# omkuprin7/ldpc-simulator

Hardware: AMD Instinct MI355X
Metric: decoded codewords/s + info-bits/s at fixed (N, rate, max_iter, Eb/N0) (higher is better)
Workload: dtype f64

## Files before the change

### ldpc-simulator_amd/csrc/ldpc_api.cpp

```cpp
#include <hip/hip_runtime.h>

#include <algorithm>
#include <cfloat>
#include <climits>
#include <cstdarg>
#include <cstdio>
#include <cstring>
#include <mutex>
#include <string>
#include <vector>

#include "ldpc_internal.h"
#include "mc_stats_host.h"
#include "rate_match_host.h"
#include "spa_device.h"

using ldpc::DevGraph;
using ldpc::DevState;
using ldpc::PhysRule;
using ldpc::PhysTile;
using ldpc::kTile;

static thread_local std::string g_last_error;

// ... 65 lines not shown
    uint32_t *ord_keys = nullptr;
    int *ord_vals = nullptr, *ord = nullptr;
    int64_t ord_cap = 0;
    void *ord_tmp = nullptr;
    size_t ord_tmp_bytes = 0;
    DevState st{};
    bool ms_on = false;
    int ms_max_failed = 0;
    unsigned long long *ms_buf = nullptr;
    size_t ms_words = 0;
    long long *ms_slots = nullptr;
    int *ms_tile = nullptr;
    int ms_state = 0;
    int ms_points = 0, ms_T = 0, ms_run_failed = 0;
    ldpc::FrameChannel chan{};
    std::vector<int32_t> rm_punct, rm_short;
    ldpc::RateMatchTables rm_tab;
    uint32_t *rm_dev = nullptr;
    bool rm_stale = false;
    bool prof = false;
    struct Span {
        int kind;
        hipEvent_t a, b;
    };
    std::vector<Span> spans;
    std::vector<hipEvent_t> pool;
};

namespace {

constexpr size_t kLdsLimit = 160 * 1024 - 1024;

int tile_scratch_rows(const DevGraph &g) { return g.ef == 8 ? ldpc::tile8_scratch_per_tile(g) : 2; }

template <int W = ldpc::kSubWaves>
std::vector<int> sub_p3_deps(int m, const int *row_ptr, const int *col_idx, bool drop_last = false) {
    std::vector<int> dep((size_t)m * W, 1);
    auto spans = [&](int r, long long lo[W], long long hi[W], bool ne[W]) {
        const int beg = row_ptr[r];
        const int deg = std::max(0, row_ptr[r + 1] - beg - (drop_last ? 1 : 0)), C = (deg + W - 1) / W;
        long long prev = -1;
        int last = -1;
        for (int w = 0; w < W; ++w) {
            const int cnt = std::max(0, std::min(deg - w * C, C));
            ne[w] = cnt > 0;
            if (!ne[w]) continue;
            lo[w] = prev + 1;
            hi[w] = prev = col_idx[beg + w * C + cnt - 1];
            last = w;
        }
        if (last >= 0) hi[last] = LLONG_MAX;
        return last >= 0;
    };
    long long plo[W], phi[W], lo[W], hi[W];
    bool pne[W], ne[W];
    bool prev_any = m > 0 && spans(0, plo, phi, pne);
    for (int r = 1; r < m; ++r) {
        spans(r, lo, hi, ne);
        for (int w = 0; w < W; ++w) {
            if (!ne[w]) continue;
            int vlo = W, vhi = -1;
            for (int v = 0; v < W; ++v)
                if (!prev_any || (pne[v] && plo[v] <= hi[w] && lo[w] <= phi[v])) {
                    vlo = std::min(vlo, v);
                    vhi = std::max(vhi, v);
                }
// ... 1 lines not shown
        }
        std::copy(lo, lo + W, plo);
        std::copy(hi, hi + W, phi);
        std::copy(ne, ne + W, pne);
        prev_any = std::any_of(ne, ne + W, [](bool b) { return b; });
    }
    return dep;
}

int require_gpu() {
    int n = 0;
    if (hipGetDeviceCount(&n) != hipSuccess || n <= 0)
        return ldpc_fail(LDPC_EDEVICE, "no HIP device visible: the SPA decoder runs only on the GPU");
    return LDPC_OK;
}

template <class T>
int dev_alloc(T **p, size_t count) {
    *p = nullptr;
    if (count == 0) return LDPC_OK;
    hipError_t e = hipMalloc((void **)p, count * sizeof(T));
    if (e != hipSuccess) {
        *p = nullptr;
        return ldpc_fail(LDPC_ENOMEM, "hipMalloc(%zu bytes) failed: %s", count * sizeof(T), hipGetErrorString(e));
    }
    return LDPC_OK;
}

int ensure_messages(ldpc_decoder *d) {
    if (d->E) return LDPC_OK;
    const DevGraph &G = d->g->dg;
    const size_t cap = (size_t)d->cap_tiles * kTile;
    int rc = dev_alloc(&d->E, cap * (size_t)G.nnz + (size_t)ldpc::kEPadEdges * kTile);
    if (!rc) rc = dev_alloc(&d->T, (size_t)d->nslots * G.max_row_deg * kTile);
    if (rc) {
        (void)hipFree(d->E);
        d->E = nullptr;
    }
    return rc;
}

int ensure_pbits(ldpc_decoder *d, const DevGraph &P) {
    if (d->pbits) return LDPC_OK;
    const size_t mw = (size_t)(P.m + 31) / 32, mw32 = (mw + 31) / 32;
    return dev_alloc(&d->pbits, (size_t)d->cap_tiles * (mw + mw32) * kTile);
}

int ensure_phys_tile(ldpc_decoder *d, const DevGraph &P) {
    const size_t cap = (size_t)d->cap_tiles * kTile;
    const int64_t need = (int64_t)(cap * (size_t)P.nnz);
    if (d->pE_cap < need) {
        (void)hipFree(d->pE);
        d->pE = nullptr;
        d->pE_cap = 0;
        if (int rc = dev_alloc(&d->pE, (size_t)need)) return rc;
        d->pE_cap = need;
    }
    if (!d->pL && dev_alloc(&d->pL, cap * (size_t)d->g->dg.n)) return LDPC_ENOMEM;
    if (!d->pLam && dev_alloc(&d->pLam, cap * (size_t)d->g->dg.n)) return LDPC_ENOMEM;
    if (!d->pbad && dev_alloc(&d->pbad, 2 * cap)) return LDPC_ENOMEM;
    if (!d->pzb && dev_alloc(&d->pzb, cap * (size_t)((d->g->dg.n + 7) / 8))) return LDPC_ENOMEM;
    return LDPC_OK;
}

PhysTile phys_tile(ldpc_decoder *d) {
    const DevGraph &G = d->g->dg;
    uint32_t *wpar = d->pbits ? d->pbits + (size_t)d->cap_tiles * ((G.m + 31) / 32) * kTile : nullptr;
// ... 183 lines not shown
        if (e == hipSuccess) {
            const bool last = it + 1 == max_iter;
            if (edge)
                e = timed(d, LDPC_K_VN_EDGE, s, [&] {
                    return ldpc::launch_vn_edge_decode(G, st, it, last, nllr, d->tzb, d->tcnt, d->tbad, s);
                });
            else if (cols)
                e = timed(d, LDPC_K_VN_COLS, s, [&] {
                    return ldpc::launch_vn_cols_decode(G, st, it, last, nllr, d->tzb, d->tcnt, s);
                });
            else
                e = timed(d, LDPC_K_VN, s, [&] { return ldpc::launch_vn(G, st, it, max_iter, nllr, s); });
        }
        if (e == hipSuccess && poll && it + 1 < max_iter && (it < 4 || (it + 1) % 4 == 0)) {
            int running = 0;
            e = hipMemcpyAsync(&running, d->pactive + it, sizeof(int), hipMemcpyDeviceToHost, s);
            if (e == hipSuccess) e = hipStreamSynchronize(s);
            if (e == hipSuccess && running == 0) break;
        }
    }
    return hip(e);
}

int scratch_slots() { return 4096; }


size_t workspace_bytes(const DevGraph &g, int cap_tiles) {
    const size_t cap = (size_t)cap_tiles * kTile;
    const size_t kw = (size_t)((g.k + 31) / 32);
    size_t b = 0;
    b += cap * (size_t)g.nnz * 8;
    const size_t slots = ldpc::use_tile(g) ? std::max(scratch_slots(), cap_tiles * tile_scratch_rows(g)) : scratch_slots();
    b += slots * g.max_row_deg * kTile * 8;
    b += 4 * (kRareHead + (size_t)cap_tiles * g.m * 4);
    b += 2 * cap * (size_t)g.n * 8;
    b += (7 * cap + cap_tiles) * 4;
    b += cap * kw * 4;
    b += 2 * cap * (size_t)g.n * 8;
    b += cap * (size_t)g.n;
    b += cap * ((size_t)(g.n + 31) / 32) * 4 + 2 * cap * 4;
    return b;
}

}

extern "C" {

const char *ldpc_last_error(void) { return g_last_error.c_str(); }
int ldpc_abi_version(void) { return LDPC_ABI_VERSION; }

int ldpc_device_count(void) {
    int n = 0;
    if (hipGetDeviceCount(&n) != hipSuccess) return 0;
    return n;
}

namespace {

int check_csr(const char *fn, int32_t m, int32_t n, const int32_t *row_ptr, const int32_t *col_idx, int *max_row,
              int *min_row) {
    if (m <= 0 || n <= 0 || m > n || !row_ptr || !col_idx)
        return ldpc_fail(LDPC_EINVAL, "%s: bad shape m=%d n=%d", fn, m, n);
    if (row_ptr[0] != 0) return ldpc_fail(LDPC_EINVAL, "%s: row_ptr[0] != 0", fn);
    const int64_t nnz = row_ptr[m];
    if (nnz <= 0 || nnz > (int64_t)(INT32_MAX / kTile) || (int64_t)n > (int64_t)(INT32_MAX / kTile))
        return ldpc_fail(LDPC_ERANGE, "%s: nnz=%lld outside 32-bit tile indexing", fn, (long long)nnz);
// ... 1728 lines not shown
```

### ldpc-simulator_amd/csrc/spa_device.h

```cpp
#pragma once
#include <hip/hip_runtime.h>
#include <cstdint>

namespace ldpc {

constexpr int kTile = 64;

constexpr int kSubWaves = 16;
constexpr int kEPadEdges = 128;

struct DevGraph {
    int m, n, k, nnz;
    int max_row_deg, max_col_deg;
    int std_form;
    int ira;
    const int *row_ptr;
    const int *col_idx;
    const int *csc_ptr;
    const int *csc_edge;
    const int *csc_row;
    const uint32_t *a_packed;
    const int *p3dep;
    const int *p3dep8;
    int ef;
// ... 32 lines not shown
    uint32_t *pbits;
    uint32_t *wpar;
    int cap;
    uint8_t *zb;
};

hipError_t launch_reset(const DevGraph &g, const DevState &st, hipStream_t s);
hipError_t launch_load_llr(const DevGraph &g, const DevState &st, const double *llr, hipStream_t s);
hipError_t launch_cn(const DevGraph &g, const DevState &st, int it, hipStream_t s, bool stream = false);
bool use_cn_row(const DevGraph &g);
hipError_t launch_cn_rare(const DevGraph &g, const DevState &st, int it, hipStream_t s, bool stream = false);
hipError_t launch_vn(const DevGraph &g, const DevState &st, int it, int max_iter, bool nllr, hipStream_t s,
                     unsigned long long *stream_ctr = nullptr);
size_t tile_lds_bytes(const DevGraph &g);
const char *tile_kernel_name(const DevGraph &g);
bool use_tile(const DevGraph &g);
hipError_t launch_tile(const DevGraph &g, const DevState &st, int max_iter, bool nllr, hipStream_t s);
bool use_tile_stream(const DevGraph &g);
hipError_t launch_tile_stream(const DevGraph &g, const DevState &st, int max_iter, bool nllr, uint64_t seed,
                              int snr_point, double sigma, int64_t frame0, int64_t total, unsigned long long *next,
                              unsigned long long *ctr, int64_t handoff, hipStream_t s);
bool tile8_applies(const DevGraph &g);
bool tile8_pair_fits(const DevGraph &g);
size_t tile8_lds_bytes(const DevGraph &g);
int tile8_scratch_per_tile(const DevGraph &g);
hipError_t launch_tile8(const DevGraph &g, const DevState &st, int max_iter, bool nllr, hipStream_t s);
size_t tile8_stream_lds_bytes(const DevGraph &g);
hipError_t launch_tile8_stream(const DevGraph &g, const DevState &st, int max_iter, bool nllr, uint64_t seed,
                               int snr_point, double sigma, int64_t frame0, int64_t total, unsigned long long *next,
                               unsigned long long *ctr, int64_t handoff, hipStream_t s);
size_t tile64_lds_bytes(const DevGraph &g);
int sub_frames(const DevGraph &g);
size_t sub_lds_bytes(const DevGraph &g);
hipError_t launch_tile_sub(const DevGraph &g, const DevState &st, int max_iter, bool nllr, hipStream_t s);
hipError_t launch_tile_sub_stream(const DevGraph &g, const DevState &st, int max_iter, bool nllr, uint64_t seed,
                                  int snr_point, double sigma, int64_t frame0, int64_t total,
                                  unsigned long long *next, unsigned long long *ctr, int64_t handoff, hipStream_t s);
hipError_t launch_stream_init(const DevGraph &g, const DevState &st, hipStream_t s);
hipError_t launch_vn_tail(const DevGraph &g, const DevState &st, int max_iter, bool nllr, uint32_t *zb, int *cnt,
                          unsigned long long *ctr, hipStream_t s);
hipError_t launch_vn_cols_decode(const DevGraph &g, const DevState &st, int it, bool last, bool nllr, uint32_t *zb,
                                 int *cnt, hipStream_t s);
hipError_t launch_tail_exit_decode(const DevGraph &g, const DevState &st, int it, bool last, bool nllr, uint32_t *zb,
                                   int *cnt, int *gbad, hipStream_t s);
int edge_max_deg();
hipError_t launch_cn_edge(const DevGraph &g, const DevState &st, int it, hipStream_t s);
hipError_t launch_vn_edge_decode(const DevGraph &g, const DevState &st, int it, bool last, bool nllr, uint32_t *zb,
                                 int *cnt, int *gbad, hipStream_t s);
int cn_sub_shape(const DevGraph &g);
hipError_t launch_cn_sub(const DevGraph &g, const DevState &st, int it, hipStream_t s, bool stream);
__host__ __device__ inline uint32_t rare_code(int tile_row, uint32_t subs) {
    return (uint32_t)tile_row | (subs << 28);
}
size_t frame_order_temp_bytes(int total);
hipError_t launch_frame_order(const DevGraph &g, uint64_t seed, int snr_point, double sigma, int64_t frame0,
                              int total, uint32_t *keys, int *vals, int *order, void *temp, size_t temp_bytes,
                              hipStream_t s);
__device__ __forceinline__ long long supply_frame(const DevState &st, int64_t frame0, int64_t idx) {
    return (long long)(frame0 + (st.order ? (int64_t)st.order[idx] : idx));
}
hipError_t launch_refill(const DevGraph &g, const DevState &st, uint64_t seed, int snr_point, double sigma,
                         int64_t frame0, int64_t total, unsigned long long *next, hipStream_t s);
hipError_t launch_compact(const DevGraph &g, const DevState &st, int nt, int cap, int *pairs, hipStream_t s);
hipError_t launch_compact_plan(const DevState &st, int nt, int cap, int *pairs, hipStream_t s);
hipError_t launch_finalize(const DevGraph &g, const DevState &st, uint8_t *z, double *post,
                           hipStream_t s);
// ... 166 lines not shown
```

### ldpc-simulator_amd/csrc/tile_sub.hip

```cpp
#include <hip/hip_runtime.h>

#include <cstdint>
#include <cstdlib>

#include "cn_common.h"
#include "frame_source.h"
#include "spa_device.h"
#include "spa_math.h"
#include "tile_common.h"

namespace ldpc {
namespace {

constexpr int kSW = kSubWaves;
#ifdef LDPC_SUB_TIMERS
#define SUB_NT 7
#define SUB_STAMP(v) const uint64_t v = __builtin_amdgcn_s_memtime()
#define SUB_ADD(c, i, a, b) ((c).tm[i] += (b) - (a))
#else
#define SUB_STAMP(v)
#define SUB_ADD(c, i, a, b)
#endif
constexpr size_t kSubLdsMax = 163840;


template <int Q>
struct SubCfg {
    static constexpr int F = kTile / Q;
    static constexpr int K = Q == 4 ? 10 : 8;
};

constexpr int kSR = 4;
__device__ __forceinline__ int sub_wave(int hw) { return (hw & 3) * (kSW / 4) + (hw >> 2); }
typedef unsigned int sub_u2 __attribute__((ext_vector_type(2)));
constexpr uint32_t kSubOOB = 0xfffffff0u;
__device__ __forceinline__ void st_sub_msg(__amdgpu_buffer_rsrc_t r, uint32_t off, double v) {
    __builtin_amdgcn_raw_buffer_store_b64(__builtin_bit_cast(sub_u2, v), r, off, 0, 2 );
}
__device__ __forceinline__ double ld_sub_msg(__amdgpu_buffer_rsrc_t r, uint32_t off) {
    return __builtin_bit_cast(double, __builtin_amdgcn_raw_buffer_load_b64(r, off, 0, 2 ));
}
__device__ __forceinline__ __amdgpu_buffer_rsrc_t sub_rsrc(const void *base, size_t bytes) {
    return __builtin_amdgcn_make_buffer_rsrc(const_cast<void *>(base), (short)0, (int)min(bytes, (size_t)0x7fffffff),
                                            0x00020000);
}

constexpr int kCRing = 3;
struct SubLayout {
    size_t S, math, slot, zb, ib, lane_i, flags, dummy, cidx, total;
// ... 36 lines not shown
    c.cnt = max(0, min(c.deg - wave * C, C));
    c.CS = (C + Q - 1) / Q;
    return c;
}

template <int Q>
struct SubCtx {
    static constexpr int F = SubCfg<Q>::F;
    static constexpr int K = SubCfg<Q>::K;
    const int *__restrict__ col_idx;
    const int *__restrict__ row_ptr;
    double *Eb;
    double *Lb;
    const double *Cb;
    double *Tb;
    size_t tbuf;
    double *S;
    double *dummy;
    double *slot;
    uint32_t *ib;
    uint16_t *cidx;
    int m;
    int *flag, *tinyf, *tseq, *p3row;
    const int *p3dep;
    LdsTanh ttab;
    LdsAtanh ltab;
    AtanhCoef ac;
    bool coef_arg;
    const char *Eu, *Lu, *Cu;
    __amdgpu_buffer_rsrc_t rE;
    uint32_t lo8;
    int k, wave, j, f;
    int ep0;
    bool first, live;
    bool fresh;
    bool verify;
    bool prove;
    int *mdiff;
    int ntiny;
#ifdef LDPC_SUB_TIMERS
    mutable uint64_t tm[SUB_NT];
#endif
};

template <int Q>
__device__ __forceinline__ int sub_nj(const SubCtx<Q> &c, const SubChunk &rc) {
    return max(0, min(rc.cnt - c.j * rc.CS, rc.CS));
}
template <int Q>
__device__ __forceinline__ int sub_edge(const SubCtx<Q> &c, const SubChunk &rc, int i) {
    return rc.c0 + min(c.j * rc.CS + i, rc.cnt - 1);
}
template <int Q>
__device__ __forceinline__ uint32_t sub_off(const SubCtx<Q> &c, int item) {
    return ((uint32_t)item << 9) + c.lo8;
}
template <int Q>
__device__ __forceinline__ double *sub_l(const SubCtx<Q> &c, int col) {
    return (double *)(c.Lu + sub_off(c, col));
}
template <int Q>
__device__ __forceinline__ const double *sub_c(const SubCtx<Q> &c, int col) {
    return (const double *)(c.Cu + sub_off(c, col));
}
template <int Q>
__device__ __forceinline__ int sub_col(const SubCtx<Q> &c, int edge) {
    return *(const int *)((const char *)c.col_idx + ((uint32_t)edge << 2));
}
template <int Q>
__device__ __forceinline__ const uint16_t *sub_lcols(const SubCtx<Q> &c, int r, const SubChunk &rc) {
    return c.cidx + (r % kCRing) * kSW * Q * SubCfg<Q>::K + c.j * rc.CS;
}
template <int Q>
__device__ __forceinline__ uint32_t sub_eoff(const SubCtx<Q> &c, const SubChunk &rc) {
    return ((uint32_t)(rc.c0 + c.j * rc.CS) << 9) + c.lo8;
}
template <int Q>
__device__ __forceinline__ int sub_stage_issue(const SubCtx<Q> &c, int q) {
    const SubChunk rc = sub_chunk(c.row_ptr, min(q, c.m - 1), c.wave, Q);
    const int L = threadIdx.x & 63;
    return sub_col(c, min(max(rc.c0 + min(L, rc.cnt - 1), 0), c.row_ptr[c.m] - 1));
}
template <int Q>
__device__ __forceinline__ void sub_stage_commit(const SubCtx<Q> &c, int q, int v) {
    if (q >= c.m) return;
    constexpr int W = Q * SubCfg<Q>::K;
    __builtin_amdgcn_fence(__ATOMIC_RELEASE, "wavefront");
    if ((int)(threadIdx.x & 63) < W) c.cidx[(q % kCRing) * kSW * W + (threadIdx.x & 63)] = (uint16_t)v;
    __builtin_amdgcn_fence(__ATOMIC_ACQUIRE, "wavefront");
}

template <int Q>
__device__ __forceinline__ bool sub_p1(const SubCtx<Q> &c, int r, const SubChunk &rc, double (&t)[SubCfg<Q>::K]) {
    constexpr int K = SubCfg<Q>::K;
    bool tiny = false;
    const int sv = sub_stage_issue(c, r + 1);
    if (rc.cnt > 0 && c.first) {
        const int njt = c.live ? sub_nj(c, rc) : 0;
        const uint16_t *lc = sub_lcols(c, r, rc);
        int col[K];
#pragma unroll
        for (int i = 0; i < K; ++i) col[i] = lc[i];
#pragma unroll
        for (int i = 0; i < K; ++i) t[i] = ld_l2((const double *)(c.Lu + sub_off(c, col[i])));
#pragma unroll
        for (int i = 0; i < K; ++i) {
            tiny |= i < njt && !(fabs(t[i]) > kTiny);
            t[i] = i < njt ? t[i] : 1.0;
        }
    } else if (rc.cnt > 0) {
        const int nj = sub_nj(c, rc);
        const int njt = c.live ? nj : 0;
        const uint16_t *lc = sub_lcols(c, r, rc);
        const uint32_t eoff = sub_eoff(c, rc);
        const bool noE = c.fresh;
        int col[K];
        double eo[K];
#pragma unroll
        for (int i = 0; i < K; ++i) {
            eo[i] = ld_sub_msg(c.rE, noE ? kSubOOB : eoff + (uint32_t)i * (kTile * sizeof(double)));
            col[i] = lc[i];
        }
#pragma unroll
        for (int i = 0; i < K; ++i) t[i] = ld_l2((const double *)(c.Lu + sub_off(c, col[i])));
#pragma unroll
        for (int i = 0; i < K; ++i) {
            const double M = noE ? t[i] : t[i] - eo[i];
            const double d = M * 0.5;
            double th[1] = {dfrom(dbits(fmin(fabs(d), 17.5)) | (dbits(d) & 0x8000000000000000ull))};
            np_tanh_n<1, LdsTanh, true>(th, c.ttab);
            const double tv = th[0];
            tiny |= i < njt && !(fabs(tv) > kTiny);
            t[i] = i < nj ? tv : 1.0;
        }
    }
    sub_stage_commit(c, r + 1, sv);
    return __ballot(tiny) != 0ull;
}

template <int Q>
__device__ __forceinline__ void sub_tanh_table(const SubCtx<Q> &c, int n, int me, int nthr) {
    for (int col = me; col < n; col += nthr) {
        const double d = *sub_c(c, col) * 0.5;
        double th[1] = {dfrom(dbits(fmin(fabs(d), 17.5)) | (dbits(d) & 0x8000000000000000ull))};
        np_tanh_n<1, LdsTanh, true>(th, c.ttab);
        if (c.live) *sub_l(c, col) = th[0];
    }
}

__device__ __forceinline__ uint32_t p16(uint32_t x, int which) {
    const auto r = __builtin_amdgcn_permlane16_swap(x, x, false, false);
    return which ? r[1] : r[0];
}
__device__ __forceinline__ uint32_t p32(uint32_t x, int which) {
    const auto r = __builtin_amdgcn_permlane32_swap(x, x, false, false);
    return which ? r[1] : r[0];
}
__device__ __forceinline__ double group_up4(double v, int jj) {
    const uint64_t u = dbits(v);
    uint32_t lo = (uint32_t)u, hi = (uint32_t)(u >> 32);
    if (jj == 1) {
        lo = p16(p32(lo, 0), 1);
        hi = p16(p32(hi, 0), 1);
    } else {
        lo = p16(lo, 0);
        hi = p16(hi, 0);
    }
    return dfrom(((uint64_t)hi << 32) | lo);
}


template <int K, int N>
struct SubMul {
    static __device__ __forceinline__ double run(double P, const double (&t)[K], int n) {
        if (n == N) {
#pragma unroll
            for (int i = 0; i < N; ++i) P = P * t[i];
            return P;
        }
// ... 35 lines not shown
#pragma unroll
        for (int jj = 0; jj < Q; ++jj) {
            if (jj * rc.CS < rc.cnt) {
                const double Pl = SubMul<K, K>::run(P, t, rc.CS);
                last = jj;
                if (jj + 1 < Q && (jj + 1) * rc.CS < rc.cnt)
                    P = group_up4(Pl, jj);
                else
                    P = Pl;
            }
        }
    }
    if ((threadIdx.x & 63) == 0) {
        if (c.wave == 0)
            lds_st(c.tinyf + s, tiny ? 1 : 0);
        else if (tiny)
            lds_st(c.tinyf + s, 1);
    }
    if (c.j == last) *sl = P;
    lds_release();
    if ((threadIdx.x & 63) == 0) lds_st(c.flag + s, ep + c.wave + 1);
    __builtin_amdgcn_s_setprio(0);
    SUB_STAMP(h2);
    SUB_ADD(c, 1, h1, h2);
}

template <int Q>
__device__ __forceinline__ void sub_order(const SubCtx<Q> &c, int r) {
    if (r > 0) {
        const int d = ld_table(c.p3dep, r * kSW + c.wave);
        for (int v = d & 0xff; v <= (d >> 8); ++v) wait_ge<false>(c.p3row + v, r);
    }
}
template <int Q>
__device__ __forceinline__ void sub_p3_body(SubCtx<Q> &c, int r, double (&t)[SubCfg<Q>::K]) {
    constexpr int F = SubCfg<Q>::F, K = SubCfg<Q>::K;
    const SubChunk rc = sub_chunk(c.row_ptr, r, c.wave, Q);
    if (rc.deg == 0) return;
    const int s = r & (kSR - 1);
    const int ep = ((c.ep0 + r) & 0x3ffffff) * 32;
    const double chI = *sub_c(c, c.k + r);
    SUB_STAMP(q0);
    wait_flag<false>(c.flag + s, ep + kSW);
    SUB_STAMP(q1);
    SUB_ADD(c, 2, q0, q1);
    const bool tiny_row = uniform(lds_ld(c.tinyf + s)) != 0;
    if (rc.cnt == 0) {
        sub_order(c, r);
        if (tiny_row) {
            c.ntiny += 1;
            if ((threadIdx.x & 63) == 0)
                __hip_atomic_fetch_add(c.tseq, 1, __ATOMIC_RELEASE, __HIP_MEMORY_SCOPE_WORKGROUP);
            wait_flag<false>(c.tseq, c.ntiny * kSW);
        }
        return;
    }
    const double P = c.slot[s * F];
    const int nj = sub_nj(c, rc);
    const uint16_t *lc = sub_lcols(c, r, rc);
    int col[K];
#pragma unroll
    for (int i = 0; i < K; ++i)
        col[i] = lc[i];
    if (!tiny_row) {
        bool big = false;
        const double lim = c.live ? kAtanhIdent : INFINITY;
        if (div_nr_ok(c.live ? P : 1.0)) {
#pragma unroll
            for (int i = 0; i < K; ++i)
                if (i < rc.CS) {
                    t[i] = div_nr(P, t[i]);
                    big |= !(fabs(t[i]) < lim);
                }
        } else {
#pragma unroll
            for (int i = 0; i < K; ++i)
                if (i < rc.CS) {
                    t[i] = P / t[i];
                    big |= !(fabs(t[i]) < lim);
                }
        }
        if (__ballot(big) == 0ull) {
#pragma unroll
            for (int i = 0; i < K; ++i)
                if (i < rc.CS) t[i] = 2.0 * t[i];
        } else {
            const AtanhCoef ac = c.coef_arg ? c.ac : coef_load();
#pragma unroll
            for (int i = 0; i < K; ++i)
                if (i < rc.CS) t[i] = 2.0 * atanh_f(clip_cl(t[i]), c.ltab, ac);
// ... 45 lines not shown
            constexpr int H = (K + 1) / 2;
            bool nx = false;
            const bool open = c.prove && d && (lds_ld(c.mdiff + (threadIdx.x & (F - 1))) & 6) == 0;
            if (__ballot(open) != 0ull) {
#pragma unroll
                for (int h = 0; h < K; h += H) {
                    __builtin_amdgcn_sched_barrier(0);
                    double lo[H];
#pragma unroll
                    for (int i = 0; i < H; ++i)
                        lo[i] = ld_l2((const double *)(c.Lu + sub_off(c, col[min(h + i, K - 1)])));
#pragma unroll
                    for (int i = 0; i < H; ++i)
                        if (h + i < K) {
                            const int q = h + i;
                            nx |= q < njv && dbits(lo[i] - eold[q]) != dbits(lo[i] - t[q]);
                            nx |= q < njv && col[q] >= c.k && dbits(chI + (0.0 + t[q])) != dbits(lo[i]);
                        }
                }
            }
#pragma unroll
            for (int i = 0; i < K; ++i) {
                const bool di = i < njv && dbits(eold[i]) != dbits(t[i]);
                st_sub_msg(c.rE, di ? eoff + (uint32_t)i * (kTile * sizeof(double)) : kSubOOB, t[i]);
            }
            if (d) atomicOr((uint32_t *)c.mdiff + (threadIdx.x & (F - 1)), (nx || !open) ? 3u : 1u);
            if (__ballot(nx) != 0ull && (threadIdx.x & 63) < F) atomicOr((uint32_t *)c.mdiff + (threadIdx.x & 63), 4u);
        }
    } else {
        const uint32_t eoff = sub_eoff(c, rc);
#pragma unroll
        for (int i = 0; i < K; ++i)
            st_sub_msg(c.rE, (i < nj && c.live) ? eoff + (uint32_t)i * (kTile * sizeof(double)) : kSubOOB, t[i]);
    }
    double EnI = 0.0;
    int colI = -1;
    double *sp[K];
#pragma unroll
    for (int i = 0; i < K; ++i) {
        const bool own = i < nj;
        const bool a = own && col[i] < c.k;
        sp[i] = a ? c.S + (size_t)col[i] * F : c.dummy;
        if (own && !a) {
            EnI = t[i];
            colI = col[i];
        }
    }
    SUB_STAMP(q2);
    SUB_ADD(c, 3, q1, q2);
    sub_order(c, r);
    SUB_STAMP(q3);
    SUB_ADD(c, 4, q2, q3);
#pragma unroll
    for (int i = 0; i < K; ++i)
        __hip_atomic_fetch_add(sp[i], t[i], __ATOMIC_RELAXED, __HIP_MEMORY_SCOPE_WORKGROUP);
    if (colI >= 0) {
        const double Lj = chI + (0.0 + EnI);
        if (c.live) *sub_l(c, colI) = Lj;
        if (!(Lj < 0.0)) {
            const int q = colI - c.k;
            atomicOr(c.ib + (q >> 5) * F, 1u << (q & 31));
        }
    }
    SUB_STAMP(q4);
    SUB_ADD(c, 5, q3, q4);
}

template <int Q>
__device__ __forceinline__ void sub_p3(SubCtx<Q> &c, int r, double (&t)[SubCfg<Q>::K]) {
    sub_p3_body<Q>(c, r, t);
    lds_release();
    if ((threadIdx.x & 63) == 0)
        lds_st(c.p3row + c.wave, r + 1);
}
__device__ __forceinline__ void sub_p3_reset(int *p3row) {
    if (threadIdx.x < kSW) p3row[threadIdx.x] = 0;
}
__device__ __forceinline__ int sub_epoch0(int pass, int m) {
    return (int)(((uint32_t)pass * (uint32_t)m) & 0x3ffffffu);
}

template <int Q>
__device__ __forceinline__ void sub_body(SubCtx<Q> &c, int r, int m, double (&tcur)[SubCfg<Q>::K], bool ycur,
                                         double (&toth)[SubCfg<Q>::K], bool &yoth) {
    if (r < m) sub_hop(c, r, tcur, ycur);
    if (r >= 1) sub_p3<Q>(c, r - 1, toth);
    SUB_STAMP(p0);
    if (r + 1 < m) yoth = sub_p1<Q>(c, r + 1, sub_chunk(c.row_ptr, r + 1, c.wave, Q), toth);
    SUB_STAMP(p1);
    SUB_ADD(c, 6, p0, p1);
}

template <int Q>
__global__ __launch_bounds__(64 * kSW, 1) void tile_sub_kernel(DevGraph g, DevState st, int max_iter, int nllr,
                                                               const int *__restrict__ col_idx,
                                                               const int *__restrict__ row_ptr, AtanhCoef ac, int fp) {
    constexpr int F = SubCfg<Q>::F, K = SubCfg<Q>::K;
    extern __shared__ __attribute__((aligned(16))) unsigned char lds[];
    __shared__ int pdiffl[F], mdiffl[F];
    const SubLayout ly = sub_layout(g.k, g.m, F);
    double *S = (double *)(lds + ly.S);
    MathLds &mlds = *(MathLds *)(lds + ly.math);
    uint32_t *zb = (uint32_t *)(lds + ly.zb);
    uint32_t *ib = (uint32_t *)(lds + ly.ib);
    int *bad = (int *)(lds + ly.lane_i);
    int *cntl = bad + F;
    int *livel = cntl + F;
    int *flags = (int *)(lds + ly.flags);
    const int kw = (g.k + 31) >> 5, mw = (g.m + 31) >> 5;
    const int tile = blockIdx.x / Q, sub = blockIdx.x % Q;
    if (tile >= st.ntiles) return;

    fill_math_lds(mlds);
    for (int i = threadIdx.x; i < g.k * F; i += blockDim.x) S[i] = 0.0;
    for (int i = threadIdx.x; i < (kw + mw) * F; i += blockDim.x) zb[i] = 0u;
    for (int i = threadIdx.x; i < 2 * F; i += blockDim.x) bad[i] = 0;
    if (threadIdx.x < 2 * kSR) flags[threadIdx.x] = -1;
    if (threadIdx.x >= 2 * kSR && threadIdx.x < 2 * kSR + 2 + kSW) flags[threadIdx.x] = 0;
    const int lane = threadIdx.x & 63;
    const int wave = uniform(sub_wave(threadIdx.x >> 6));
    const int j = lane / F, f = lane % F;
    const int fr = tile * kTile + sub * F + f;
    if (wave == 0 && j == 0) {
        livel[f] = st.done[fr] == 0 ? 1 : 0;
        pdiffl[f] = 0;
        mdiffl[f] = 0;
    }
    __syncthreads();
    if (!st.tile_active[tile]) return;
// ... 10 lines not shown
    const size_t lo = (size_t)sub * F + f;
    c.Eb = st.E + (size_t)tile * g.nnz * kTile + lo;
    c.Lb = st.L + (size_t)tile * g.n * kTile + lo;
    c.Cb = st.ch + (size_t)tile * g.n * kTile + lo;
    c.Eu = (const char *)(st.E + (size_t)tile * g.nnz * kTile);
    c.rE = sub_rsrc(c.Eu, (size_t)g.nnz * kTile * sizeof(double));
    c.Lu = (const char *)(st.L + (size_t)tile * g.n * kTile);
    c.Cu = (const char *)(st.ch + (size_t)tile * g.n * kTile);
    c.lo8 = (uint32_t)lo * 8u;
    c.Tb = st.T + (size_t)blockIdx.x * 2 * g.max_row_deg * F + f;
    c.tbuf = (size_t)g.max_row_deg * F;
    c.S = S + f;
    c.dummy = (double *)(lds + ly.dummy) + f;
    c.slot = (double *)(lds + ly.slot) + f;
    c.ib = ib + f;
    c.cidx = (uint16_t *)(lds + ly.cidx) + wave * Q * K;
    c.m = g.m;
    c.flag = flags;
    c.tinyf = flags + kSR;
    c.tseq = flags + 2 * kSR;
    c.p3row = flags + 2 * kSR + 2;
    c.p3dep = g.p3dep;
    c.ttab = LdsTanh{mlds.tanh};
    c.ltab = LdsAtanh{mlds.atanh};
    c.coef_arg = false;
    c.ac = ac;
    c.k = g.k;
    c.wave = wave;
    c.j = j;
    c.f = f;
    c.ntiny = 0;
    c.fresh = false;
    c.mdiff = mdiffl;
#ifdef LDPC_SUB_TIMERS
    for (int i = 0; i < SUB_NT; ++i) c.tm[i] = 0;
#endif
    const int m = g.m;
    const int nthr = kSW * Q;
    const int me = wave * Q + j;

    int ctl = 1, vnext = 1, vgap = 1;
    const bool fpn = (fp & 2) != 0;
    if (max_iter > 0) {
        c.live = livel[f] != 0;
        sub_tanh_table<Q>(c, g.n, me, nthr);
        __builtin_amdgcn_fence(__ATOMIC_RELEASE, "agent");
        __syncthreads();
    }
    for (int it = 0; it < max_iter; ++it) {
        c.first = it == 0;
        c.live = livel[f] != 0;
        c.ep0 = sub_epoch0(it, m);
        const bool verify = fp != 0 && it >= vnext && (ctl & 2) != 0;
        c.verify = verify;
        c.prove = verify && fpn;
        double tA[K], tB[K];
        bool yA = false, yB = false;
        if (m > 0) {
            sub_stage_commit(c, 0, sub_stage_issue(c, 0));
            yA = sub_p1<Q>(c, 0, sub_chunk(row_ptr, 0, wave, Q), tA);
        }
        for (int r = 0; r <= m; r += 2) {
            sub_body<Q>(c, r, m, tA, yA, tB, yB);
            if (r + 1 <= m) sub_body<Q>(c, r + 1, m, tB, yB, tA, yA);
        }
        __syncthreads();
        sub_p3_reset(c.p3row);

        int my_cnt = 0;
        bool pd = false;
        for (int col = me; col < g.k; col += nthr) {
            double *sp = c.S + (size_t)col * F;
            const double Sj = *sp;
            *sp = 0.0;
            const double chj = *sub_c(c, col);
            const double Lj = chj + Sj;
            if (nllr || fp) {
                const double ap = c.first ? chj : ld_l2(sub_l(c, col));
                if (nllr) my_cnt += (fabs(Lj) <= 7.0 && ap * Lj < 0.0) ? 1 : 0;
                pd |= dbits(ap) != dbits(Lj);
            }
            if (c.live) *sub_l(c, col) = Lj;
            if (!(Lj < 0.0)) atomicOr(zb + (col >> 5) * F + f, 1u << (col & 31));
        }
        if (nllr && my_cnt) atomicAdd(cntl + f, my_cnt);
        if (fp && pd && c.live) atomicOr((uint32_t *)pdiffl + f, 1u);
        __syncthreads();

        uint32_t acc = 0u;
        for (int r = me; r < m; r += nthr) {
            const uint32_t *ar = g.a_packed + (size_t)r * kw;
            uint32_t par = ib[(r >> 5) * F + f] >> (r & 31);
            for (int w = 0; w < kw; ++w) par += __builtin_popcount(ar[w] & zb[w * F + f]);
            acc |= par & 1u;
        }
        if (acc) atomicOr((uint32_t *)bad + f, 1u);
        __syncthreads();

        if (wave == 0) {
            bool still = false, fixed = false, proven = false;
            if (j == 0 && c.live) {
                if (nllr) {
                    const int cn = cntl[f];
                    st.nllr_cnt[fr] = cn;
                    if (st.nllr_hist)
                        st.nllr_hist[(size_t)fr * st.hist_stride + it] = g.k > 0 ? (double)cn / g.k : 0.0;
                }
                if (bad[f] == 0) {
                    st.done[fr] = 1;
                    st.conv[fr] = it;
                    st.status[fr] = 0;
// ... 14 lines not shown
                    proven = mdiffl[f] != 0;
                } else {
                    still = true;
                }
            }
            const unsigned long long any = __ballot(still);
            const unsigned long long trig = __ballot(still && fp && pdiffl[f] == 0);
            const int nfix = __popcll(__ballot(fixed));
            const unsigned long long nprv = __ballot(proven);
            if (j == 0) {
                livel[f] = still ? 1 : 0;
                bad[f] = 0;
                cntl[f] = 0;
                pdiffl[f] = 0;
                mdiffl[f] = 0;
            }
            if (lane == 0) {
                flags[2 * kSR + 1] = (any != 0ull ? 1 : 0) | (trig != 0ull ? 2 : 0) | (nfix ? 4 : 0) | (nprv != 0ull ? 8 : 0);
                if (nfix) {
                    atomicAdd(&st.fp_count[0], (unsigned long long)nfix);
                    atomicAdd(&st.fp_count[1], (unsigned long long)nfix * (unsigned long long)(max_iter - 1 - it));
                }
            }
        }
        for (int i = threadIdx.x; i < (kw + mw) * F; i += blockDim.x) zb[i] = 0u;
        __syncthreads();
        ctl = uniform(flags[2 * kSR + 1]);
        if (!(ctl & 1)) break;
        if (verify && !(ctl & 4)) {
            vnext = it + 1 + vgap;
            vgap *= 2;
        }
    }
    count_rare_rows(st, c.tseq, kSW);
#ifdef LDPC_SUB_TIMERS
    if ((blockIdx.x == 0 || blockIdx.x == 777) && (threadIdx.x & 63) == 0)
        printf("SUB b=%d w=%d hopw=%llu hop=%llu p3f=%llu p3m=%llu p3o=%llu p3s=%llu p1=%llu\n", (int)blockIdx.x,
               c.wave, (unsigned long long)c.tm[0], (unsigned long long)c.tm[1], (unsigned long long)c.tm[2],
               (unsigned long long)c.tm[3], (unsigned long long)c.tm[4], (unsigned long long)c.tm[5],
               (unsigned long long)c.tm[6]);
#endif
}

template <int Q>
__global__ __launch_bounds__(64 * kSW, 1) void tile_sub_stream_kernel(
    DevGraph g, DevState st, int max_iter, int nllr, const int *__restrict__ col_idx,
    const int *__restrict__ row_ptr, AtanhCoef ac, uint64_t seed, int snr_point, double sigma, int64_t frame0,
    int64_t total, unsigned long long *next, unsigned long long *ctr, int64_t handoff) {
    constexpr int F = SubCfg<Q>::F, K = SubCfg<Q>::K;
    extern __shared__ __attribute__((aligned(16))) unsigned char lds[];
    __shared__ int itl[F], freshl[F];
    __shared__ long long gidx[F];
    __shared__ int nref;
    const SubLayout ly = sub_layout(g.k, g.m, F);
    double *S = (double *)(lds + ly.S);
    MathLds &mlds = *(MathLds *)(lds + ly.math);
    uint32_t *zb = (uint32_t *)(lds + ly.zb);
    uint32_t *ib = (uint32_t *)(lds + ly.ib);
    int *bad = (int *)(lds + ly.lane_i);
    int *cntl = bad + F;
    int *livel = cntl + F;
    int *flags = (int *)(lds + ly.flags);
    const int kw = (g.k + 31) >> 5, mw = (g.m + 31) >> 5;
    const int tile = blockIdx.x / Q, sub = blockIdx.x % Q;
    if (tile >= st.ntiles) return;

    fill_math_lds(mlds);
    for (int i = threadIdx.x; i < g.k * F; i += blockDim.x) S[i] = 0.0;
    for (int i = threadIdx.x; i < (kw + mw) * F; i += blockDim.x) zb[i] = 0u;
    for (int i = threadIdx.x; i < 2 * F; i += blockDim.x) bad[i] = 0;
    if (threadIdx.x < 2 * kSR) flags[threadIdx.x] = -1;
    if (threadIdx.x >= 2 * kSR && threadIdx.x < 2 * kSR + 2 + kSW) flags[threadIdx.x] = 0;
    const int lane = threadIdx.x & 63;
    const int wave = uniform(sub_wave(threadIdx.x >> 6));
// ... 11 lines not shown
    c.col_idx = col_idx;
    c.row_ptr = row_ptr;
    const size_t lo = (size_t)lane64;
    c.Eb = st.E + (size_t)tile * g.nnz * kTile + lo;
    c.Lb = st.L + (size_t)tile * g.n * kTile + lo;
    c.Cb = st.ch + (size_t)tile * g.n * kTile + lo;
    c.Eu = (const char *)(st.E + (size_t)tile * g.nnz * kTile);
    c.rE = sub_rsrc(c.Eu, (size_t)g.nnz * kTile * sizeof(double));
    c.Lu = (const char *)(st.L + (size_t)tile * g.n * kTile);
    c.Cu = (const char *)(st.ch + (size_t)tile * g.n * kTile);
    c.lo8 = (uint32_t)lo * 8u;
    c.Tb = st.T + (size_t)blockIdx.x * 2 * g.max_row_deg * F + f;
    c.tbuf = (size_t)g.max_row_deg * F;
    c.S = S + f;
    c.dummy = (double *)(lds + ly.dummy) + f;
    c.slot = (double *)(lds + ly.slot) + f;
    c.ib = ib + f;
    c.cidx = (uint16_t *)(lds + ly.cidx) + wave * Q * K;
    c.m = g.m;
    c.flag = flags;
    c.tinyf = flags + kSR;
    c.tseq = flags + 2 * kSR;
    c.p3row = flags + 2 * kSR + 2;
    c.p3dep = g.p3dep;
    c.ttab = LdsTanh{mlds.tanh};
    c.ltab = LdsAtanh{mlds.atanh};
    c.coef_arg = kStreamCoefArg;
    c.ac = ac;
    c.k = g.k;
    c.wave = wave;
    c.j = j;
    c.f = f;
    c.ntiny = 0;
    c.first = false;
    c.verify = false;
    c.prove = false;
    c.mdiff = nullptr;
    const int m = g.m;
    const int nthr = kSW * Q;
    const int me = wave * Q + j;
    const uint32_t *Ut = st.ubits + (size_t)tile * kw * kTile + lane64;

    for (int pass = 0;; ++pass) {
        if (wave == 0) {
            int stop = 0;
            if (handoff > 0 && lane == 0) {
                const long long nx = (long long)__hip_atomic_load(next, __ATOMIC_RELAXED, __HIP_MEMORY_SCOPE_AGENT);
                const long long fin = (long long)__hip_atomic_load(ctr, __ATOMIC_RELAXED, __HIP_MEMORY_SCOPE_AGENT);
                stop = nx >= total && total - fin <= handoff ? 1 : 0;
            }
            stop = uniform(stop);
            if (stop) want = false;
            const unsigned long long w = __ballot(want);
            bool have = false;
            if (w != 0ull) {
                const int first = __ffsll((long long)w) - 1;
                unsigned long long base = 0ull;
                if (lane == first) base = atomicAdd(next, (unsigned long long)__popcll(w));
                base = __shfl(base, first);
                const unsigned long long below = lane ? (w & (~0ull >> (64 - lane))) : 0ull;
                const int64_t idx = (int64_t)(base + (unsigned long long)__popcll(below));
                have = want && idx < total;
                if (slot_lane) gidx[f] = have ? supply_frame(st, frame0, idx) : -1ll;
                if (want) {
                    livel[f] = have ? 1 : 0;
                    freshl[f] = have ? 1 : 0;
                    itl[f] = 0;
// ... 108 lines not shown
template <int Q>
size_t sub_lds_bytes_q(const DevGraph &g) {
    constexpr int F = SubCfg<Q>::F, K = SubCfg<Q>::K;
    if (!g.std_form || !g.a_packed || g.k <= 0 || g.max_row_deg > kSW * Q * K || Q * K > 64 || g.n > 65535)
        return 0;
    const size_t b = sub_layout(g.k, g.m, F).total;
    return b + 2 * F * sizeof(int) <= kSubLdsMax ? b : 0;
}

}

int sub_frames(const DevGraph &g) { return sub_lds_bytes_q<4>(g) ? 16 : 0; }
size_t sub_lds_bytes(const DevGraph &g) { return sub_lds_bytes_q<4>(g); }

hipError_t launch_tile_sub_stream(const DevGraph &g, const DevState &st, int max_iter, bool nllr, uint64_t seed,
                                  int snr_point, double sigma, int64_t frame0, int64_t total,
                                  unsigned long long *next, unsigned long long *ctr, int64_t handoff, hipStream_t s) {
    const size_t lds = sub_lds_bytes_q<4>(g);
    if (!lds || !g.a_packed || !st.ubits || 2 * st.ntiles > st.nslots ||
        lds + 2 * 16 * sizeof(int) + 16 * sizeof(long long) + 16 > kSubLdsMax)
        return hipErrorInvalidValue;
    tile_sub_stream_kernel<4><<<st.ntiles * 4, 64 * kSW, lds, s>>>(g, st, max_iter, nllr ? 1 : 0, g.col_idx, g.row_ptr,
                                                                   kAtanhCoef, seed, snr_point, sigma, frame0, total,
                                                                   next, ctr, handoff);
    return hipGetLastError();
}

hipError_t launch_tile_sub(const DevGraph &g, const DevState &st, int max_iter, bool nllr, hipStream_t s) {
    const size_t lds = sub_lds_bytes(g);
    if (!lds || 2 * st.ntiles > st.nslots) return hipErrorInvalidValue;
    const char *e = getenv("LDPC_FIXED_POINT");
    const char *en = getenv("LDPC_FP_NEXT");
    const int fp = (!e || atoi(e) != 0) ? (1 | ((!en || atoi(en) != 0) ? 2 : 0)) : 0;
    tile_sub_kernel<4><<<st.ntiles * 4, 64 * kSW, lds, s>>>(g, st, max_iter, nllr ? 1 : 0, g.col_idx, g.row_ptr,
                                                            kAtanhCoef, fp);
    return hipGetLastError();
}

}
```

Before: 125,800.

## Split first decoder iteration into a pass0 kernel with row-product prepass

Adds a separate pass0 kernel that runs iteration 0 of the sub-tile decoder. Before the row sweep, a prepass computes per-row products of tanh values and rare-row flags into a global scratch area. Iteration 0 then consumes these precomputed products through a specialized row loop that skips the flag waits and overlaps the next row's loads with the current row's stores. The main kernel resumes from iteration 1 using a control handoff value stored in global memory. This costs an extra kernel launch, additional global scratch allocation, and more code paths that must stay numerically consistent with the original.

```diff
diff --git a/ldpc-simulator_amd/csrc/ldpc_api.cpp b/ldpc-simulator_amd/csrc/ldpc_api.cpp
--- a/ldpc-simulator_amd/csrc/ldpc_api.cpp
+++ b/ldpc-simulator_amd/csrc/ldpc_api.cpp
@@ -121,6 +121,9 @@
 constexpr size_t kLdsLimit = 160 * 1024 - 1024;
 
 int tile_scratch_rows(const DevGraph &g) { return g.ef == 8 ? ldpc::tile8_scratch_per_tile(g) : 2; }
+size_t sub_p0_total(const DevGraph &g, int cap_tiles) {
+    return g.ef == kTile && ldpc::sub_frames(g) == 16 ? (size_t)cap_tiles * 4 * ldpc::sub_p0_doubles(g.m) : 0;
+}
 
 template <int W = ldpc::kSubWaves>
 std::vector<int> sub_p3_deps(int m, const int *row_ptr, const int *col_idx, bool drop_last = false) {
@@ -188,7 +191,7 @@
     const DevGraph &G = d->g->dg;
     const size_t cap = (size_t)d->cap_tiles * kTile;
     int rc = dev_alloc(&d->E, cap * (size_t)G.nnz + (size_t)ldpc::kEPadEdges * kTile);
-    if (!rc) rc = dev_alloc(&d->T, (size_t)d->nslots * G.max_row_deg * kTile);
+    if (!rc) rc = dev_alloc(&d->T, (size_t)d->nslots * G.max_row_deg * kTile + sub_p0_total(G, d->cap_tiles));
     if (rc) {
         (void)hipFree(d->E);
         d->E = nullptr;
@@ -438,6 +441,7 @@
     b += cap * (size_t)g.nnz * 8;
     const size_t slots = ldpc::use_tile(g) ? std::max(scratch_slots(), cap_tiles * tile_scratch_rows(g)) : scratch_slots();
     b += slots * g.max_row_deg * kTile * 8;
+    b += sub_p0_total(g, cap_tiles) * 8;
     b += 4 * (kRareHead + (size_t)cap_tiles * g.m * 4);
     b += 2 * cap * (size_t)g.n * 8;
     b += (7 * cap + cap_tiles) * 4;
diff --git a/ldpc-simulator_amd/csrc/spa_device.h b/ldpc-simulator_amd/csrc/spa_device.h
--- a/ldpc-simulator_amd/csrc/spa_device.h
+++ b/ldpc-simulator_amd/csrc/spa_device.h
@@ -88,6 +88,10 @@
 size_t tile64_lds_bytes(const DevGraph &g);
 int sub_frames(const DevGraph &g);
 size_t sub_lds_bytes(const DevGraph &g);
+__host__ __device__ inline size_t sub_p0_doubles(int m) { return (size_t)m * 16 + ((size_t)m + 2) / 2; }
+__host__ __device__ inline double *sub_p0(const DevGraph &g, const DevState &st) {
+    return st.T + (size_t)st.nslots * g.max_row_deg * kTile;
+}
 hipError_t launch_tile_sub(const DevGraph &g, const DevState &st, int max_iter, bool nllr, hipStream_t s);
 hipError_t launch_tile_sub_stream(const DevGraph &g, const DevState &st, int max_iter, bool nllr, uint64_t seed,
                                   int snr_point, double sigma, int64_t frame0, int64_t total,
diff --git a/ldpc-simulator_amd/csrc/tile_sub.hip b/ldpc-simulator_amd/csrc/tile_sub.hip
--- a/ldpc-simulator_amd/csrc/tile_sub.hip
+++ b/ldpc-simulator_amd/csrc/tile_sub.hip
@@ -14,7 +14,7 @@
 
 constexpr int kSW = kSubWaves;
 #ifdef LDPC_SUB_TIMERS
-#define SUB_NT 7
+#define SUB_NT 8
 #define SUB_STAMP(v) const uint64_t v = __builtin_amdgcn_s_memtime()
 #define SUB_ADD(c, i, a, b) ((c).tm[i] += (b) - (a))
 #else
@@ -117,7 +117,9 @@
     uint32_t lo8;
     int k, wave, j, f;
     int ep0;
-    bool first, live;
+    double *P0;
+    int *R;
+    bool live;
     bool fresh;
     bool verify;
     bool prove;
@@ -180,20 +182,7 @@
     constexpr int K = SubCfg<Q>::K;
     bool tiny = false;
     const int sv = sub_stage_issue(c, r + 1);
-    if (rc.cnt > 0 && c.first) {
-        const int njt = c.live ? sub_nj(c, rc) : 0;
-        const uint16_t *lc = sub_lcols(c, r, rc);
-        int col[K];
-#pragma unroll
-        for (int i = 0; i < K; ++i) col[i] = lc[i];
-#pragma unroll
-        for (int i = 0; i < K; ++i) t[i] = ld_l2((const double *)(c.Lu + sub_off(c, col[i])));
-#pragma unroll
-        for (int i = 0; i < K; ++i) {
-            tiny |= i < njt && !(fabs(t[i]) > kTiny);
-            t[i] = i < njt ? t[i] : 1.0;
-        }
-    } else if (rc.cnt > 0) {
+    if (rc.cnt > 0) {
         const int nj = sub_nj(c, rc);
         const int njt = c.live ? nj : 0;
         const uint16_t *lc = sub_lcols(c, r, rc);
@@ -230,6 +219,60 @@
         double th[1] = {dfrom(dbits(fmin(fabs(d), 17.5)) | (dbits(d) & 0x8000000000000000ull))};
         np_tanh_n<1, LdsTanh, true>(th, c.ttab);
         if (c.live) *sub_l(c, col) = th[0];
+        if (col < c.k) c.S[(size_t)col * SubCfg<Q>::F] = c.live ? th[0] : 1.0;
+    }
+}
+
+constexpr int kPU = 8;
+template <int Q>
+__device__ __forceinline__ void sub_prepass(const SubCtx<Q> &c, int hw, int nnz, const double *one) {
+    constexpr int F = SubCfg<Q>::F;
+    const unsigned long long gmask = ((1ull << F) - 1ull) << (c.j * F);
+    const __amdgpu_buffer_rsrc_t rC = sub_rsrc(c.col_idx, (size_t)nnz * sizeof(int));
+    for (int b = 0; b < c.m; b += kSW * Q) {
+        const int r = b + hw * Q + c.j;
+        const bool in = r < c.m;
+        const int beg = in ? c.row_ptr[r] : 0;
+        const int deg = in ? c.row_ptr[r + 1] - beg : 0;
+        int dmax = 0;
+#pragma unroll
+        for (int jj = 0; jj < Q; ++jj) dmax = max(dmax, __shfl(deg, jj * F));
+        dmax = uniform(dmax);
+        const int voff = beg * 4;
+        int colA[kPU], colB[kPU];
+#pragma unroll
+        for (int u = 0; u < kPU; ++u) colA[u] = __builtin_amdgcn_raw_buffer_load_b32(rC, voff + 4 * u, 0, 0);
+        const int lastcol = deg > 0 ? sub_col(c, beg + deg - 1) : 0;
+        const double tI = ld_l2(sub_l(c, lastcol));
+        const bool idl = deg > 0 && lastcol >= c.k;
+        const int degA = deg - (idl ? 1 : 0);
+        double P = 1.0;
+        bool vote = false;
+        auto step = [&](const int (&cur)[kPU], int (&nxt)[kPU], int e0) {
+            const int vo = voff + 4 * (e0 + kPU);
+#pragma unroll
+            for (int u = 0; u < kPU; ++u) nxt[u] = __builtin_amdgcn_raw_buffer_load_b32(rC, vo + 4 * u, 0, 0);
+            double tv[kPU];
+#pragma unroll
+            for (int u = 0; u < kPU; ++u) tv[u] = *(e0 + u < degA ? c.S + (size_t)cur[u] * F : one);
+#pragma unroll
+            for (int u = 0; u < kPU; ++u) {
+                vote |= !(fabs(tv[u]) > kTiny);
+                P = P * tv[u];
+            }
+        };
+        for (int e0 = 0; e0 < dmax; e0 += 2 * kPU) {
+            step(colA, colB, e0);
+            step(colB, colA, e0 + kPU);
+        }
+        const double tl = idl && c.live ? tI : 1.0;
+        vote |= !(fabs(tl) > kTiny);
+        P = P * tl;
+        const bool rare = (__ballot(vote) & gmask) != 0ull;
+        if (in) {
+            c.P0[(size_t)r * F] = P;
+            if (c.f == 0) c.R[r] = rare ? 1 : 0;
+        }
     }
 }
 
@@ -331,19 +374,23 @@
         for (int v = d & 0xff; v <= (d >> 8); ++v) wait_ge<false>(c.p3row + v, r);
     }
 }
-template <int Q>
-__device__ __forceinline__ void sub_p3_body(SubCtx<Q> &c, int r, double (&t)[SubCfg<Q>::K]) {
+struct SubNoHook {
+    __device__ __forceinline__ void operator()() const {}
+};
+template <int Q, bool kPre = false, class Hook = SubNoHook>
+__device__ __forceinline__ void sub_p3_body(SubCtx<Q> &c, int r, double (&t)[SubCfg<Q>::K], double Ppre = 0.0,
+                                            bool rare_pre = false, Hook after_stores = Hook{}) {
     constexpr int F = SubCfg<Q>::F, K = SubCfg<Q>::K;
     const SubChunk rc = sub_chunk(c.row_ptr, r, c.wave, Q);
-    if (rc.deg == 0) return;
+    if (!kPre && rc.deg == 0) return;
     const int s = r & (kSR - 1);
     const int ep = ((c.ep0 + r) & 0x3ffffff) * 32;
     const double chI = *sub_c(c, c.k + r);
     SUB_STAMP(q0);
-    wait_flag<false>(c.flag + s, ep + kSW);
+    if constexpr (!kPre) wait_flag<false>(c.flag + s, ep + kSW);
     SUB_STAMP(q1);
     SUB_ADD(c, 2, q0, q1);
-    const bool tiny_row = uniform(lds_ld(c.tinyf + s)) != 0;
+    const bool tiny_row = kPre ? rare_pre : uniform(lds_ld(c.tinyf + s)) != 0;
     if (rc.cnt == 0) {
         sub_order(c, r);
         if (tiny_row) {
@@ -352,9 +399,14 @@
                 __hip_atomic_fetch_add(c.tseq, 1, __ATOMIC_RELEASE, __HIP_MEMORY_SCOPE_WORKGROUP);
             wait_flag<false>(c.tseq, c.ntiny * kSW);
         }
+        if constexpr (kPre) {
+#pragma unroll
+            for (int i = 0; i < K; ++i) st_sub_msg(c.rE, kSubOOB, 0.0);
+            after_stores();
+        }
         return;
     }
-    const double P = c.slot[s * F];
+    const double P = kPre ? Ppre : c.slot[s * F];
     const int nj = sub_nj(c, rc);
     const uint16_t *lc = sub_lcols(c, r, rc);
     int col[K];
@@ -466,6 +518,7 @@
 #pragma unroll
         for (int i = 0; i < K; ++i)
             st_sub_msg(c.rE, (i < nj && c.live) ? eoff + (uint32_t)i * (kTile * sizeof(double)) : kSubOOB, t[i]);
+        after_stores();
     }
     double EnI = 0.0;
     int colI = -1;
@@ -501,6 +554,51 @@
 }
 
 template <int Q>
+__device__ __forceinline__ void sub_g0(const SubCtx<Q> &c, int r, double (&t)[SubCfg<Q>::K], double &P, int &rare) {
+    constexpr int F = SubCfg<Q>::F, K = SubCfg<Q>::K;
+    const SubChunk rc = sub_chunk(c.row_ptr, r, c.wave, Q);
+    P = ld_l2(c.P0 + (size_t)r * F);
+    rare = __hip_atomic_load(c.R + r, __ATOMIC_RELAXED, __HIP_MEMORY_SCOPE_AGENT);
+    const uint16_t *lc = sub_lcols(c, r, rc);
+    int col[K];
+#pragma unroll
+    for (int i = 0; i < K; ++i) col[i] = lc[i];
+#pragma unroll
+    for (int i = 0; i < K; ++i) t[i] = ld_l2((const double *)(c.Lu + sub_off(c, col[i])));
+}
+template <int Q>
+__device__ __forceinline__ void sub_body0(SubCtx<Q> &c, int r, int m, double (&tcur)[SubCfg<Q>::K], const double &Pcur,
+                                          int ycur, double (&toth)[SubCfg<Q>::K], double &Poth, int &yoth, int &sv) {
+    constexpr int K = SubCfg<Q>::K;
+    const SubChunk rc = sub_chunk(c.row_ptr, r, c.wave, Q);
+    const int njt = c.live ? sub_nj(c, rc) : 0;
+#pragma unroll
+    for (int i = 0; i < K; ++i) tcur[i] = i < njt ? tcur[i] : 1.0;
+    sub_p3_body<Q, true>(c, r, tcur, Pcur, uniform(ycur) != 0, [&]() {
+        sub_stage_commit(c, r + 1, sv);
+        sv = sub_stage_issue(c, r + 2);
+        sub_g0<Q>(c, min(r + 1, m - 1), toth, Poth, yoth);
+    });
+    lds_release();
+    if ((threadIdx.x & 63) == 0) lds_st(c.p3row + c.wave, r + 1);
+}
+template <int Q>
+__device__ __forceinline__ void sub_rows0(SubCtx<Q> &c, int m) {
+    constexpr int K = SubCfg<Q>::K;
+    if (m <= 0) return;
+    double tA[K], tB[K];
+    double PA = 1.0, PB = 1.0;
+    int yA = 0, yB = 0;
+    sub_stage_commit(c, 0, sub_stage_issue(c, 0));
+    int sv = sub_stage_issue(c, 1);
+    sub_g0<Q>(c, 0, tA, PA, yA);
+    for (int r = 0; r < m; r += 2) {
+        sub_body0<Q>(c, r, m, tA, PA, yA, tB, PB, yB, sv);
+        if (r + 1 < m) sub_body0<Q>(c, r + 1, m, tB, PB, yB, tA, PA, yA, sv);
+    }
+}
+
+template <int Q>
 __device__ __forceinline__ void sub_p3(SubCtx<Q> &c, int r, double (&t)[SubCfg<Q>::K]) {
     sub_p3_body<Q>(c, r, t);
     lds_release();
@@ -525,10 +623,10 @@
     SUB_ADD(c, 6, p0, p1);
 }
 
-template <int Q>
-__global__ __launch_bounds__(64 * kSW, 1) void tile_sub_kernel(DevGraph g, DevState st, int max_iter, int nllr,
-                                                               const int *__restrict__ col_idx,
-                                                               const int *__restrict__ row_ptr, AtanhCoef ac, int fp) {
+template <int Q, bool kPass0>
+__device__ __forceinline__ void tile_sub_run(const DevGraph &g, const DevState &st, int max_iter, int nllr,
+                                             const int *__restrict__ col_idx, const int *__restrict__ row_ptr,
+                                             const AtanhCoef &ac, int fp) {
     constexpr int F = SubCfg<Q>::F, K = SubCfg<Q>::K;
     extern __shared__ __attribute__((aligned(16))) unsigned char lds[];
     __shared__ int pdiffl[F], mdiffl[F];
@@ -605,6 +703,10 @@
     c.ntiny = 0;
     c.fresh = false;
     c.mdiff = mdiffl;
+    c.P0 = sub_p0(g, st) + (size_t)blockIdx.x * sub_p0_doubles(g.m);
+    c.R = (int *)(c.P0 + (size_t)g.m * F);
+    c.P0 += f;
+    int *hand = c.R + g.m;
 #ifdef LDPC_SUB_TIMERS
     for (int i = 0; i < SUB_NT; ++i) c.tm[i] = 0;
 #endif
@@ -614,28 +716,42 @@
 
     int ctl = 1, vnext = 1, vgap = 1;
     const bool fpn = (fp & 2) != 0;
-    if (max_iter > 0) {
+    if constexpr (!kPass0) ctl = uniform(__hip_atomic_load(hand, __ATOMIC_RELAXED, __HIP_MEMORY_SCOPE_AGENT));
+    if (kPass0 && max_iter > 0) {
+        SUB_STAMP(pp0);
         c.live = livel[f] != 0;
+        double *one = (double *)(lds + ly.slot);
+        if (threadIdx.x < F) one[threadIdx.x] = 1.0;
         sub_tanh_table<Q>(c, g.n, me, nthr);
         __builtin_amdgcn_fence(__ATOMIC_RELEASE, "agent");
         __syncthreads();
-    }
-    for (int it = 0; it < max_iter; ++it) {
-        c.first = it == 0;
+        sub_prepass<Q>(c, (int)(threadIdx.x >> 6), g.nnz, one + f);
+        __builtin_amdgcn_fence(__ATOMIC_RELEASE, "agent");
+        __syncthreads();
+        for (int i = threadIdx.x; i < g.k * F; i += blockDim.x) S[i] = 0.0;
+        __syncthreads();
+        SUB_STAMP(pp1);
+        SUB_ADD(c, 7, pp0, pp1);
+    }
+    for (int it = kPass0 ? 0 : 1; it < (kPass0 ? min(max_iter, 1) : max_iter); ++it) {
         c.live = livel[f] != 0;
         c.ep0 = sub_epoch0(it, m);
-        const bool verify = fp != 0 && it >= vnext && (ctl & 2) != 0;
+        const bool verify = !kPass0 && fp != 0 && it >= vnext && (ctl & 2) != 0;
         c.verify = verify;
         c.prove = verify && fpn;
-        double tA[K], tB[K];
-        bool yA = false, yB = false;
-        if (m > 0) {
-            sub_stage_commit(c, 0, sub_stage_issue(c, 0));
-            yA = sub_p1<Q>(c, 0, sub_chunk(row_ptr, 0, wave, Q), tA);
-        }
-        for (int r = 0; r <= m; r += 2) {
-            sub_body<Q>(c, r, m, tA, yA, tB, yB);
-            if (r + 1 <= m) sub_body<Q>(c, r + 1, m, tB, yB, tA, yA);
+        if constexpr (kPass0) {
+            sub_rows0<Q>(c, m);
+        } else {
+            double tA[K], tB[K];
+            bool yA = false, yB = false;
+            if (m > 0) {
+                sub_stage_commit(c, 0, sub_stage_issue(c, 0));
+                yA = sub_p1<Q>(c, 0, sub_chunk(row_ptr, 0, wave, Q), tA);
+            }
+            for (int r = 0; r <= m; r += 2) {
+                sub_body<Q>(c, r, m, tA, yA, tB, yB);
+                if (r + 1 <= m) sub_body<Q>(c, r + 1, m, tB, yB, tA, yA);
+            }
         }
         __syncthreads();
         sub_p3_reset(c.p3row);
@@ -649,7 +765,7 @@
             const double chj = *sub_c(c, col);
             const double Lj = chj + Sj;
             if (nllr || fp) {
-                const double ap = c.first ? chj : ld_l2(sub_l(c, col));
+                const double ap = kPass0 ? chj : ld_l2(sub_l(c, col));
                 if (nllr) my_cnt += (fabs(Lj) <= 7.0 && ap * Lj < 0.0) ? 1 : 0;
                 pd |= dbits(ap) != dbits(Lj);
             }
@@ -730,14 +846,28 @@
             vgap *= 2;
         }
     }
+    if (kPass0 && threadIdx.x == 0) *hand = ctl;
     count_rare_rows(st, c.tseq, kSW);
 #ifdef LDPC_SUB_TIMERS
     if ((blockIdx.x == 0 || blockIdx.x == 777) && (threadIdx.x & 63) == 0)
-        printf("SUB b=%d w=%d hopw=%llu hop=%llu p3f=%llu p3m=%llu p3o=%llu p3s=%llu p1=%llu\n", (int)blockIdx.x,
+        printf("SUB b=%d w=%d hopw=%llu hop=%llu p3f=%llu p3m=%llu p3o=%llu p3s=%llu p1=%llu pre=%llu\n", (int)blockIdx.x,
                c.wave, (unsigned long long)c.tm[0], (unsigned long long)c.tm[1], (unsigned long long)c.tm[2],
                (unsigned long long)c.tm[3], (unsigned long long)c.tm[4], (unsigned long long)c.tm[5],
-               (unsigned long long)c.tm[6]);
+               (unsigned long long)c.tm[6], (unsigned long long)c.tm[7]);
 #endif
+}
+template <int Q>
+__global__ __launch_bounds__(64 * kSW, 1) void tile_sub_kernel(DevGraph g, DevState st, int max_iter, int nllr,
+                                                               const int *__restrict__ col_idx,
+                                                               const int *__restrict__ row_ptr, AtanhCoef ac, int fp) {
+    tile_sub_run<Q, false>(g, st, max_iter, nllr, col_idx, row_ptr, ac, fp);
+}
+template <int Q>
+__global__ __launch_bounds__(64 * kSW, 1) void tile_sub_pass0_kernel(DevGraph g, DevState st, int max_iter, int nllr,
+                                                                     const int *__restrict__ col_idx,
+                                                                     const int *__restrict__ row_ptr, AtanhCoef ac,
+                                                                     int fp) {
+    tile_sub_run<Q, true>(g, st, max_iter, nllr, col_idx, row_ptr, ac, fp);
 }
 
 template <int Q>
@@ -815,7 +945,8 @@
     c.j = j;
     c.f = f;
     c.ntiny = 0;
-    c.first = false;
+    c.P0 = nullptr;
+    c.R = nullptr;
     c.verify = false;
     c.prove = false;
     c.mdiff = nullptr;
@@ -990,6 +1121,10 @@
     const char *e = getenv("LDPC_FIXED_POINT");
     const char *en = getenv("LDPC_FP_NEXT");
     const int fp = (!e || atoi(e) != 0) ? (1 | ((!en || atoi(en) != 0) ? 2 : 0)) : 0;
+    tile_sub_pass0_kernel<4><<<st.ntiles * 4, 64 * kSW, lds, s>>>(g, st, max_iter, nllr ? 1 : 0, g.col_idx, g.row_ptr,
+                                                                  kAtanhCoef, fp);
+    const hipError_t e0 = hipGetLastError();
+    if (e0 != hipSuccess || max_iter <= 1) return e0;
     tile_sub_kernel<4><<<st.ntiles * 4, 64 * kSW, lds, s>>>(g, st, max_iter, nllr ? 1 : 0, g.col_idx, g.row_ptr,
                                                             kAtanhCoef, fp);
     return hipGetLastError();
```

Result: no change. 125,500 (-0.2%).
